# snipsco/sda

Measured on AMD Instinct MI355X. Metric: share-gen + clerk-sum elements/sec (mod q), higher is better.
Workload: dtype u64

## Files before the change

### sda_amd/csrc/clerk_sum.hpp

```cpp
#pragma once
#include <stddef.h>
#include <stdint.h>
#include <hip/hip_runtime.h>

#include "modarith.hpp"

namespace sda {

typedef long long ll2 __attribute__((ext_vector_type(2)));

template <bool VEC, int UNROLL>
__device__ __forceinline__ void combine_pair(uint64_t* __restrict__ acc_lo, int64_t* __restrict__ acc_hi,
                                             const int64_t* __restrict__ shares, size_t job_stride, size_t n_rows,
                                             size_t row_stride, size_t dimension, size_t rows_per_split, bool atomic,
                                             size_t pair, size_t by, size_t bz) {
    const size_t c0 = 2 * pair;
    if (c0 >= dimension) return;
    const bool two = c0 + 1 < dimension;
    const size_t job = by;
    const size_t r_begin = bz * rows_per_split;
    size_t r_end = r_begin + rows_per_split;
    if (r_end > n_rows) r_end = n_rows;
    const int64_t* base = shares + job * job_stride + c0;

    uint64_t lo0 = 0, lo1 = 0;
    int64_t hi0 = 0, hi1 = 0;
    size_t r = r_begin;
    if (VEC && two) {
        for (; r + UNROLL <= r_end; r += UNROLL) {
            ll2 v[UNROLL];
#pragma unroll
            for (int u = 0; u < UNROLL; ++u)
                v[u] = __builtin_nontemporal_load(reinterpret_cast<const ll2*>(base + (r + u) * row_stride));
#pragma unroll
            for (int u = 0; u < UNROLL; ++u) { acc_add(lo0, hi0, v[u].x); acc_add(lo1, hi1, v[u].y); }
        }
        for (; r < r_end; ++r) {
            ll2 v = __builtin_nontemporal_load(reinterpret_cast<const ll2*>(base + r * row_stride));
            acc_add(lo0, hi0, v.x); acc_add(lo1, hi1, v.y);
        }
    } else {
        for (; r < r_end; ++r) {
            acc_add(lo0, hi0, base[r * row_stride]);
            if (two) acc_add(lo1, hi1, base[r * row_stride + 1]);
        }
    }

    const size_t idx = job * dimension + c0;
    if (atomic) {
        acc_atomic_add(acc_lo + idx, acc_hi + idx, lo0, hi0);
        if (two) acc_atomic_add(acc_lo + idx + 1, acc_hi + idx + 1, lo1, hi1);
    } else {
        uint64_t l = acc_lo[idx]; int64_t h = acc_hi[idx];
        uint64_t nl = l + lo0; h += hi0 + (nl < l ? 1 : 0);
        acc_lo[idx] = nl; acc_hi[idx] = h;
        if (two) {
            l = acc_lo[idx + 1]; h = acc_hi[idx + 1];
            nl = l + lo1; h += hi1 + (nl < l ? 1 : 0);
            acc_lo[idx + 1] = nl; acc_hi[idx + 1] = h;
        }
    }
}

}
```

### sda_amd/csrc/modarith.hpp

```cpp
#pragma once
#include <stdint.h>

#if defined(__HIPCC__)
#include <hip/hip_runtime.h>
#define SDA_HD __host__ __device__ __forceinline__
#define SDA_D __device__ __forceinline__
#else
#define SDA_HD inline
#define SDA_D inline
#endif

namespace sda {

typedef unsigned __int128 u128;

struct U128 {
    uint64_t lo, hi;
};

SDA_HD U128 mul64x64(uint64_t a, uint64_t b) {
#if defined(__HIP_DEVICE_COMPILE__)
    U128 r;
    r.lo = a * b;
    r.hi = __umul64hi(a, b);
    return r;
#else
    u128 p = (u128)a * b;
    return U128{(uint64_t)p, (uint64_t)(p >> 64)};
#endif
}

SDA_HD uint64_t mulhi64(uint64_t a, uint64_t b) {
#if defined(__HIP_DEVICE_COMPILE__)
    return __umul64hi(a, b);
#else
    return (uint64_t)(((u128)a * b) >> 64);
#endif
}

SDA_HD void mac128(U128& acc, uint64_t a, uint64_t b) {
    U128 p = mul64x64(a, b);
    uint64_t lo = acc.lo + p.lo;
    acc.hi += p.hi + (lo < acc.lo ? 1u : 0u);
    acc.lo = lo;
}

struct MontCtx {
    uint64_t p;
    uint64_t pinv;
    uint64_t r2;
};

SDA_HD uint64_t mont_redc(U128 T, uint64_t p, uint64_t pinv) {
    uint64_t m = T.lo * pinv;
    uint64_t t = T.hi + mulhi64(m, p) + (T.lo != 0 ? 1u : 0u);
    return t >= p ? t - p : t;
}

SDA_HD void mont_acc_condsub(U128& acc, uint64_t p) {
    if (acc.hi >= p) acc.hi -= p;
}

SDA_HD uint64_t barrett_mod64(uint64_t v, uint64_t m, uint64_t mu) {
    uint64_t qhat = mulhi64(v, mu);
    uint64_t r = v - qhat * m;
    if (r >= m) r -= m;
    if (r >= m) r -= m;
    return r;
}

SDA_HD uint64_t canon_i64(int64_t x, uint64_t m, uint64_t mu) {
    if ((uint64_t)x < m) return (uint64_t)x;
    if (x >= 0) return barrett_mod64((uint64_t)x, m, mu);
    uint64_t mag = (uint64_t)0 - (uint64_t)x;
    uint64_t r = barrett_mod64(mag, m, mu);
    return r == 0 ? 0 : m - r;
}

SDA_HD uint64_t addmod(uint64_t a, uint64_t b, uint64_t m) {
    uint64_t s = a + b;
    return s >= m ? s - m : s;
}

SDA_HD uint64_t submod(uint64_t a, uint64_t b, uint64_t m) {
    return a >= b ? a - b : a + m - b;
}

SDA_HD uint64_t mod_i128(uint64_t lo, int64_t hi, uint64_t m, uint64_t mu) {
    bool neg = hi < 0;
    uint64_t mh = (uint64_t)hi, ml = lo;
    if (neg) {
        ml = ~ml + 1;
        mh = ~mh + (ml == 0 ? 1u : 0u);
    }
    uint64_t r = barrett_mod64(mh, m, mu);
    for (int i = 63; i >= 0; --i) {
        r = (r << 1) | ((ml >> i) & 1u);
        if (r >= m) r -= m;
    }
    return (neg && r != 0) ? m - r : r;
}

#if defined(__HIPCC__)
SDA_D void acc_add(uint64_t& lo, int64_t& hi, int64_t v) {
    const uint64_t nl = lo + (uint64_t)v;
    hi += (v >> 63) + (nl < lo ? 1 : 0);
    lo = nl;
}
SDA_D void acc_atomic_add(uint64_t* lo_p, int64_t* hi_p, uint64_t lo, int64_t hi) {
    if (lo != 0) {
        const unsigned long long old = atomicAdd(reinterpret_cast<unsigned long long*>(lo_p), (unsigned long long)lo);
        if (old + lo < old) hi += 1;
    }
    if (hi != 0) atomicAdd(reinterpret_cast<unsigned long long*>(hi_p), (unsigned long long)hi);
}
#endif

SDA_HD bool lemire_sample(uint64_t x, uint64_t m, uint64_t lemire_thr, uint64_t& out) {
    U128 pr = mul64x64(x, m);
    out = pr.hi;
    return pr.lo >= lemire_thr;
}

static constexpr uint64_t kDrbgPairedMax = 0x7F7F7Full;
SDA_HD bool drbg_paired(uint64_t m) { return m <= kDrbgPairedMax; }
SDA_HD bool lemire_pair(uint64_t x, uint32_t m, uint64_t thr2, uint32_t& ra, uint32_t& rb) {
    const uint64_t t0 = (uint64_t)(uint32_t)x * m;
    const uint64_t t1 = (uint64_t)(uint32_t)(x >> 32) * m + (t0 >> 32);
    ra = (uint32_t)(t1 >> 32);
    const uint64_t u0 = (uint64_t)(uint32_t)t0 * m;
    const uint64_t u1 = (uint64_t)(uint32_t)t1 * m + (u0 >> 32);
    rb = (uint32_t)(u1 >> 32);
    return ((u1 << 32) | (uint32_t)u0) >= thr2;
}

inline uint64_t h_mulmod(uint64_t a, uint64_t b, uint64_t m) { return (uint64_t)(((u128)a * b) % m); }

inline uint64_t h_powmod(uint64_t b, uint64_t e, uint64_t m) {
    uint64_t r = 1 % m;
    b %= m;
    while (e) {
        if (e & 1) r = h_mulmod(r, b, m);
        b = h_mulmod(b, b, m);
        e >>= 1;
    }
    return r;
}

inline bool h_invmod(uint64_t a, uint64_t m, uint64_t& out) {
    __int128 r0 = m, r1 = a % m, t0 = 0, t1 = 1;
    while (r1 != 0) {
        __int128 q = r0 / r1;
        __int128 r2 = r0 - q * r1; r0 = r1; r1 = r2;
        __int128 t2 = t0 - q * t1; t0 = t1; t1 = t2;
    }
    if (r0 != 1) return false;
    if (t0 < 0) t0 += m;
    out = (uint64_t)t0;
    return true;
}

inline uint64_t h_canon(int64_t x, uint64_t m) {
    __int128 r = (__int128)x % (__int128)m;
    if (r < 0) r += m;
    return (uint64_t)r;
}

inline uint64_t h_barrett_mu(uint64_t m) {
    return (uint64_t)((((u128)1) << 64) / m);
}

inline uint64_t h_lemire_thr(uint64_t m) {
    return (uint64_t)((((u128)1) << 64) % m);
}
inline uint64_t h_lemire_thr2(uint64_t m) {
    return drbg_paired(m) ? (uint64_t)((((u128)1) << 64) % ((u128)m * m)) : 0;
}

inline MontCtx h_mont_ctx(uint64_t p) {
    MontCtx c;
    c.p = p;
    uint64_t inv = p;
    for (int i = 0; i < 6; ++i) inv *= 2 - p * inv;
    c.pinv = (uint64_t)0 - inv;
    u128 r = (((u128)1) << 64) % p;
    c.r2 = (uint64_t)((r * r) % p);
    return c;
}

inline uint64_t h_to_mont(uint64_t x, uint64_t p) {
    return (uint64_t)((((u128)x) << 64) % p);
}

}
```

### sda_amd/csrc/ngemm_kernels.hip

```cpp
#include <hip/hip_runtime.h>
#include <stdint.h>

#include "capi_internal.hpp"
#include "chacha.hpp"
#include "clerk_sum.hpp"
#include "drbg_lane.hpp"
#include "kernels.hpp"
#include "launch_plan.hpp"
#include "modarith.hpp"

namespace sda {

typedef int ng_v4i __attribute__((ext_vector_type(4)));
typedef unsigned int ng_v4u __attribute__((ext_vector_type(4)));
typedef unsigned int ng_v2u __attribute__((ext_vector_type(2)));

static constexpr int kNgCompute = 8;
static constexpr int kNgWorkers = 64 * kNgCompute;
#ifndef NG_CLERK_WAVES
#define NG_CLERK_WAVES 3
#endif
static constexpr int kNgClerkWaves = NG_CLERK_WAVES;
static constexpr int kNgThreads = kNgWorkers + 64 + 64 * kNgClerkWaves;
typedef __attribute__((address_space(3))) uint8_t* ng_lptr;
// ... 125 lines not shown
        chacha_block_lane<20>(kk, (uint32_t)I, (uint32_t)(I >> 32), (uint32_t)stream, (uint32_t)(stream >> 32) & 0xFFFFFFu, o);
        const uint32_t i0 = 2u * j, i1 = i0 + 1u;
        const bool w0 = i0 >= d_lo, w1 = i1 < d_hi;
#pragma unroll
        for (int jj = 0; jj < 8; ++jj) {
            const int cc = jj >> 1, e = jj & 1;
            const uint64_t xw = ((uint64_t)o[8 * e + cc] << 32) | o[8 * e + 4 + cc];
            uint32_t ra, rb;
            if (!lemire_pair(xw, (uint32_t)m, thr2, ra, rb)) rej |= 1ull << (8u * round + (uint32_t)jj);
            if (w0) ng_put(B, WGB, 8u * nb + jj, k + i0 - t_lo, ng_digits(ra));
            if (w1) ng_put(B, WGB, 8u * nb + jj, k + i1 - t_lo, ng_digits(rb));
        }
    }
    if (__builtin_expect(rej != 0, 0)) ng_draw_fixup<WGB>(Bt, key, stream, b0, k, t, t_lo, d_lo, cd, m, thr2, rej);
}

template <int WGB>
__device__ __noinline__ void ng_direct_pass(const uint8_t* Bt, int64_t* op, size_t stride_clerk, uint64_t b0, uint64_t batches, uint32_t k,
                                            uint32_t t_lo, uint32_t d_lo, uint32_t d_hi) {
    const uint32_t lane = threadIdx.x & 63u, wave = threadIdx.x >> 6;
    const uint32_t o_lo = (k + d_lo - t_lo) & ~3u, o_hi = k + d_hi - t_lo;
    for (uint32_t bg = 0; bg < (uint32_t)(WGB / 64); ++bg) {
        const uint32_t bl = 64u * bg + lane;
        const uint64_t b = b0 + bl;
        const __attribute__((address_space(3))) uint8_t* q = (const __attribute__((address_space(3))) uint8_t*)Bt + bl * kNgRow;
        typedef const __attribute__((address_space(3))) uint32_t* lw;
        for (uint32_t o = o_lo + 4u * wave; o < o_hi; o += 4u * (uint32_t)kNgCompute) {
            const uint32_t w0 = *(lw)(q + o);
            const uint32_t w1 = *(lw)(q + WGB * kNgRow + o);
            const uint32_t w2 = *(lw)(q + 2 * WGB * kNgRow + o);
#pragma unroll
            for (int j = 0; j < 4; ++j) {
                const uint32_t v = (uint32_t)((int32_t)(int8_t)(w0 >> (8 * j)) + 256 * (int32_t)(int8_t)(w1 >> (8 * j)) +
                                              65536 * (int32_t)(int8_t)(w2 >> (8 * j)));
                const uint32_t term = t_lo + o + (uint32_t)j;
                if (b < batches && term >= k + d_lo && term < k + d_hi)
                    __builtin_nontemporal_store((long long)v, (__attribute__((address_space(1))) long long*)(op + (size_t)(term - k) * stride_clerk + b));
            }
        }
    }
}

template <int KS, int NT, int STEP>
__device__ __forceinline__ void ng_stage(ng_v4i (&bfrag)[NT][KS > 1 ? NgBSource<KS>::in_regs : 1][3], uint8_t* Bt, uint8_t* Side, const GenLayout& L, const ModParams& mod, const DrbgKey& key,
                                         const NGemmPlan& P, const int64_t* sp, const int64_t* rp, int64_t* op, uint64_t stream, uint64_t b0,
                                         uint64_t batches
#ifdef NG_TIMING
                                         , uint64_t (&ng_tm)[4]
#endif
                                         ) {
    constexpr int WB = 16 * NT, WGB = kNgCompute * WB;
    const uint32_t lane = threadIdx.x & 63u, wave = threadIdx.x >> 6, col = lane & 15u, g = lane >> 4;
    const uint32_t k = P.k, t = P.t, kt = k + t, t_lo = 64u * STEP;
    const bool worker = wave < (uint32_t)kNgCompute;
    const bool loads = t_lo < k || rp != nullptr || t_lo + 64u > kt;
    const bool draws_here = !rp && t_lo + 64u > k && t_lo < kt;
    const uint32_t d_lo = t_lo > k ? t_lo - k : 0u, d_hi = draws_here ? (t_lo + 64u < kt ? t_lo + 64u : kt) - k : d_lo;
#ifdef NG_TIMING
    const uint64_t tq0 = __builtin_readcyclecounter();
#endif
    if (worker) {
        if (loads) ng_load_pass<WGB>(Bt, sp, rp, L.len, batches, b0, k, t, t_lo, mod.m, mod.mu);
#ifdef NG_TIMING
        ng_tm[0] += __builtin_readcyclecounter() - tq0;
#endif
        if (draws_here) ng_draw_pass<WGB>(Bt, key, stream, b0, k, t, t_lo, d_lo, d_hi - d_lo, mod.m, mod.lemire_thr2);
    }
#ifdef NG_TIMING
    const uint64_t tq1 = __builtin_readcyclecounter();
#endif
    __syncthreads();
#ifdef NG_TIMING
    const uint64_t tq2 = __builtin_readcyclecounter();
    ng_tm[1] += tq1 - tq0; ng_tm[2] += tq2 - tq1;
#endif
    if (worker) {
        if (draws_here && L.direct_rows) ng_direct_pass<WGB>(Bt, op, L.out_stride_clerk, b0, batches, k, t_lo, d_lo, d_hi);
#ifdef NG_TIMING
        ng_tm[3] += __builtin_readcyclecounter() - tq2;
#endif
        if constexpr (STEP < NgBSource<KS>::in_regs || (NgBSource<KS>::stash && STEP == KS - 2)) {
#pragma unroll
            for (int nt = 0; nt < NT; ++nt)
#pragma unroll
                for (int lb = 0; lb < 3; ++lb) {
                    const ng_v4i f = *reinterpret_cast<const ng_v4i*>(Bt + ((size_t)lb * WGB + wave * WB + NT * col + nt) * kNgRow + 16 * g);
                    if constexpr (STEP < NgBSource<KS>::in_regs) bfrag[nt][STEP][lb] = f;
                    else *reinterpret_cast<ng_v4i*>(Side + ((size_t)(wave * NT + nt) * 3 + lb) * 1024 + lane * 16) = f;
                }
        }
    }
    __syncthreads();
#ifdef NG_TIMING
    if constexpr (STEP + 1 < KS) ng_stage<KS, NT, STEP + 1>(bfrag, Bt, Side, L, mod, key, P, sp, rp, op, stream, b0, batches, ng_tm);
#else
    if constexpr (STEP + 1 < KS) ng_stage<KS, NT, STEP + 1>(bfrag, Bt, Side, L, mod, key, P, sp, rp, op, stream, b0, batches);
#endif
}

struct NgFuse {
    uint64_t* acc_lo; int64_t* acc_hi; const int64_t* prev;
    size_t job_stride, n_rows, row_stride, dimension, rows_per_split;
    uint32_t col_blocks, jobs, splits, pad;
    uint64_t n_gen, n_comb, n_comb_wg, period;
    uint64_t n_early;
    uint32_t items_per_wg;
    uint32_t pad2;
    uint64_t cw_items, cw_per_slot;
    uint64_t* cw_progress;
    uint32_t cw_col_blocks, cw_pad;
};
static constexpr int kNgClerkUnroll = 8;
static constexpr int kNgClerkUnrollShort = 20;

template <int KS> struct NgRing { static constexpr int depth = KS == 8 ? 2 : 4; };

__device__ __forceinline__ void ng_store_guard(ng_v4u v) { asm volatile("s_nop 1" ::"v"(v)); }
__device__ __forceinline__ void ng_store_guard(ng_v2u v) { asm volatile("s_nop 1" ::"v"(v)); }

struct NgClerkCursor {
    uint64_t it, end;
    uint64_t job; uint32_t bx;
    uint32_t r;
};
static constexpr int kNgClerkRows = 10;

struct NgClerkSet {
    ll2 v[kNgClerkRows];
    ll2 al, ah;
};

__device__ __forceinline__ void ng_clerk_advance(NgClerkCursor& c, uint32_t n_rows, uint32_t col_blocks) {
    c.r += kNgClerkRows;
    if (c.r >= n_rows) {
        c.r = 0; ++c.it;
        if (++c.bx == col_blocks) { c.bx = 0; ++c.job; }
    }
}
__device__ __forceinline__ void ng_clerk_load(ll2& dst, const void* p) {
    asm volatile("global_load_dwordx4 %0, %1, off nt ; NGCL" : "=v"(dst) : "v"(p) : "memory");
}
__device__ __forceinline__ void ng_clerk_load_plain(ll2& dst, const void* p) {
    asm volatile("global_load_dwordx4 %0, %1, off ; NGCL" : "=v"(dst) : "v"(p) : "memory");
}
template <int YOUNGER>
__device__ __forceinline__ void ng_clerk_wait(NgClerkSet& S) {
    static_assert(kNgClerkRows == 10, "the operand list below names ten rows");
    asm volatile("s_waitcnt vmcnt(%12) ; NGCW %0 %1 %2 %3 %4 %5 %6 %7 %8 %9 %10 %11"
                 : "+v"(S.v[0]), "+v"(S.v[1]), "+v"(S.v[2]), "+v"(S.v[3]), "+v"(S.v[4]), "+v"(S.v[5]), "+v"(S.v[6]), "+v"(S.v[7]),
                   "+v"(S.v[8]), "+v"(S.v[9]), "+v"(S.al), "+v"(S.ah)
                 : "n"(YOUNGER)
                 : "memory");
}

__device__ __forceinline__ void ng_clerk_wave(const NgFuse& F, uint64_t slot, uint32_t lane, uint32_t n_barriers, uint32_t extra) {
    if (F.cw_items == 0) {
        for (uint32_t b = 0; b < n_barriers; ++b) __builtin_amdgcn_s_barrier();
        return;
    }
    const uint32_t n_rows = (uint32_t)F.n_rows, col_blocks = F.cw_col_blocks;
    NgClerkCursor is, cs;
    is.it = slot * F.cw_per_slot < F.cw_items ? slot * F.cw_per_slot : F.cw_items;
    is.end = is.it + F.cw_per_slot < F.cw_items ? is.it + F.cw_per_slot : F.cw_items;
    is.job = is.it / col_blocks; is.bx = (uint32_t)(is.it - is.job * col_blocks); is.r = 0;
    cs = is;
    uint64_t lo0 = 0, lo1 = 0, bl0 = 0, bl1 = 0;
    int64_t hi0 = 0, hi1 = 0, bh0 = 0, bh1 = 0;
    NgClerkSet A, B;
    bool validA = false, validB = false;
    auto issue = [&](NgClerkSet& S, bool& valid) {
        valid = is.it < is.end;
        size_t c0 = 2 * ((size_t)is.bx * 64 + lane);
        if (c0 + 1 >= F.dimension) c0 = 0;
        const uint64_t job = valid ? is.job : 0;
        const uint32_t r0 = valid ? is.r : 0;
        const int64_t* base = F.prev + job * F.job_stride + c0;
        if (valid && r0 == 0) {
            const size_t idx = job * F.dimension + c0;
            ng_clerk_load_plain(S.al, F.acc_lo + idx);
            ng_clerk_load_plain(S.ah, F.acc_hi + idx);
        }
#pragma unroll
        for (int u = 0; u < kNgClerkRows; ++u) {
            const uint32_t rr = r0 + u < n_rows ? r0 + u : n_rows - 1;
            ng_clerk_load(S.v[u], base + (size_t)rr * F.row_stride);
        }
        if (valid) ng_clerk_advance(is, n_rows, col_blocks);
    };
    auto flush = [&]() {
        const size_t c0 = 2 * ((size_t)cs.bx * 64 + lane);
        if (c0 + 1 >= F.dimension) return;
        const size_t idx = cs.job * F.dimension + c0;
        const uint64_t n0 = bl0 + lo0, n1 = bl1 + lo1;
        ll2 l, h;
        l.x = (long long)n0; l.y = (long long)n1;
        h.x = bh0 + hi0 + (n0 < bl0 ? 1 : 0); h.y = bh1 + hi1 + (n1 < bl1 ? 1 : 0);
        *reinterpret_cast<ll2*>(F.acc_lo + idx) = l;
        *reinterpret_cast<ll2*>(F.acc_hi + idx) = h;
    };
    auto consume = [&](NgClerkSet& S, bool& valid) {
        if (!valid) return;
        valid = false;
        if (cs.r == 0) {
            bl0 = (uint64_t)S.al.x; bl1 = (uint64_t)S.al.y; bh0 = S.ah.x; bh1 = S.ah.y;
            lo0 = lo1 = 0; hi0 = hi1 = 0;
        }
#pragma unroll
        for (int u = 0; u < kNgClerkRows; ++u)
            if (cs.r + u < n_rows) { acc_add(lo0, hi0, S.v[u].x); acc_add(lo1, hi1, S.v[u].y); }
        if (cs.r + kNgClerkRows >= n_rows) flush();
        ng_clerk_advance(cs, n_rows, col_blocks);
    };
#pragma unroll
    for (int u = 0; u < kNgClerkRows; ++u) { A.v[u] = ll2{0, 0}; B.v[u] = ll2{0, 0}; }
    A.al = A.ah = B.al = B.ah = ll2{0, 0};
    uint32_t b = 0;
    for (; b + 1 < n_barriers; b += 2) {
        const uint32_t e = b < 32u ? (extra >> b) & 3u : 0u;
        if (e >= 1u) {
            ng_clerk_wait<kNgClerkRows>(A);
            consume(A, validA); issue(A, validA);
            ng_clerk_wait<kNgClerkRows>(B);
            consume(B, validB); issue(B, validB);
        }
        if (e >= 2u) {
            ng_clerk_wait<kNgClerkRows>(A);
            consume(A, validA); issue(A, validA);
            ng_clerk_wait<kNgClerkRows>(B);
            consume(B, validB); issue(B, validB);
        }
        ng_clerk_wait<kNgClerkRows>(A);
        consume(A, validA); issue(A, validA);
        __builtin_amdgcn_s_barrier();
        ng_clerk_wait<kNgClerkRows>(B);
        consume(B, validB); issue(B, validB);
        __builtin_amdgcn_s_barrier();
    }
    if (b < n_barriers) {
        ng_clerk_wait<kNgClerkRows>(A);
        consume(A, validA); issue(A, validA);
        __builtin_amdgcn_s_barrier();
        ng_clerk_wait<0>(B); consume(B, validB);
        ng_clerk_wait<0>(A); consume(A, validA);
    } else {
        ng_clerk_wait<0>(A); consume(A, validA);
        ng_clerk_wait<0>(B); consume(B, validB);
    }
    if (cs.it < cs.end && cs.r != 0) flush();
    if (F.cw_progress && lane == 0) { F.cw_progress[2 * slot] = cs.it; F.cw_progress[2 * slot + 1] = cs.r; }
}

static constexpr int kNgClerkRest = 16;
__global__ __launch_bounds__(64) void ngemm_clerk_rest_kernel(NgFuse F, uint64_t slots) {
    const uint32_t lane = threadIdx.x, n_rows = (uint32_t)F.n_rows;
    for (uint64_t slot = blockIdx.x; slot < slots; slot += gridDim.x) {
        uint64_t it = F.cw_progress[2 * slot];
        uint32_t r0 = (uint32_t)F.cw_progress[2 * slot + 1];
        const uint64_t first = slot * F.cw_per_slot < F.cw_items ? slot * F.cw_per_slot : F.cw_items;
        const uint64_t end = first + F.cw_per_slot < F.cw_items ? first + F.cw_per_slot : F.cw_items;
        for (; it < end; ++it, r0 = 0) {
            const uint64_t job = it / F.cw_col_blocks, bx = it - job * F.cw_col_blocks;
            const size_t c0 = 2 * ((size_t)bx * 64 + lane);
            if (c0 >= F.dimension) continue;
            const bool two = c0 + 1 < F.dimension;
            const int64_t* base = F.prev + job * F.job_stride + c0;
            const size_t idx = job * F.dimension + c0;
            const uint64_t l0 = F.acc_lo[idx], l1 = two ? F.acc_lo[idx + 1] : 0;
            const int64_t h0 = F.acc_hi[idx], h1 = two ? F.acc_hi[idx + 1] : 0;
            uint64_t lo0 = 0, lo1 = 0;
            int64_t hi0 = 0, hi1 = 0;
            for (uint32_t r = r0; r < n_rows; r += kNgClerkRest) {
                ll2 v[kNgClerkRest];
#pragma unroll
                for (int u = 0; u < kNgClerkRest; ++u) {
                    const uint32_t rr = r + u < n_rows ? r + u : n_rows - 1;
                    v[u] = __builtin_nontemporal_load(reinterpret_cast<const ll2*>(base + (size_t)rr * F.row_stride));
                }
#pragma unroll
                for (int u = 0; u < kNgClerkRest; ++u)
                    if (r + u < n_rows) { acc_add(lo0, hi0, v[u].x); if (two) acc_add(lo1, hi1, v[u].y); }
            }
            uint64_t nl = l0 + lo0;
            F.acc_lo[idx] = nl; F.acc_hi[idx] = h0 + hi0 + (nl < l0 ? 1 : 0);
            if (two) { nl = l1 + lo1; F.acc_lo[idx + 1] = nl; F.acc_hi[idx + 1] = h1 + hi1 + (nl < l1 ? 1 : 0); }
        }
    }
}

template <int N> __device__ __forceinline__ void ng_wait_vm() { asm volatile("s_waitcnt vmcnt(%0)" ::"n"(N) : "memory"); }

template <int KS>
__device__ __noinline__ void ng_loader_rows(const uint8_t* A, uint8_t* Abuf, uint32_t tiles, uint32_t lane) {
    constexpr int PIECES = KS * 3, ATILE = PIECES * 1024, DEPTH = NgRing<KS>::depth;
    auto issue_tile = [&](uint32_t tile, uint32_t slot) {
        const uint8_t* src = A + (size_t)tile * ATILE + lane * 16;
        uint8_t* dst = Abuf + slot * ATILE;
#pragma unroll
        for (int q = 0; q < PIECES; ++q)
            __builtin_amdgcn_global_load_lds((const __attribute__((address_space(1))) void*)(src + q * 1024),
                                             (__attribute__((address_space(3))) void*)(dst + q * 1024), 16, 0, 0);
    };
    uint32_t slot = DEPTH - 1;
    for (uint32_t rt = 0; rt < tiles; ++rt) {
        const uint32_t nxt = rt + DEPTH - 1;
        if (nxt < tiles) {
            issue_tile(nxt, slot);
            ng_wait_vm<PIECES * (DEPTH - 2) < 63 ? PIECES * (DEPTH - 2) : 0>();
        } else {
            ng_wait_vm<0>();
        }
        slot = slot + 1 == (uint32_t)DEPTH ? 0u : slot + 1;
        __builtin_amdgcn_s_barrier();
    }
}

template <int KS, int NT>
__global__ __launch_bounds__(kNgThreads) __attribute__((amdgpu_waves_per_eu(3, 3))) void packed_gen_ngemm_kernel(GenLayout L, ModParams mod, DrbgKey key, NGemmPlan P,
                                                                        uint64_t chunks, uint64_t batches, NgFuse F) {
    constexpr int WB = 16 * NT, WGB = kNgCompute * WB;
    constexpr int PIECES = KS * 3, ATILE = PIECES * 1024;
    constexpr int DEPTH = NgRing<KS>::depth;
    extern __shared__ __align__(16) uint8_t ng_lds[];
    uint8_t* Abuf = ng_lds;
    uint8_t* Bt = ng_lds + DEPTH * ATILE;
    uint8_t* Side = Bt + 3 * WGB * kNgRow;
    const uint32_t tid = threadIdx.x, lane = tid & 63u, wave = tid >> 6, col = lane & 15u, g = lane >> 4;
    uint64_t item = blockIdx.x;
    auto role_at = [&](uint64_t pos, uint64_t& idx) -> int {
        if (!F.n_comb_wg) { idx = pos; return pos < (uint64_t)gridDim.x ? 0 : 2; }
        const uint64_t mixed = F.n_gen + F.n_early;
        if (pos >= mixed) { idx = F.n_early + (pos - mixed); return idx < F.n_comb_wg ? 1 : 2; }
        const uint64_t q = pos / F.period, rem = pos - q * F.period;
        if (rem == 0 && q < F.n_early) { idx = q; return 1; }
        const uint64_t before = q + (rem ? 1 : 0);
        idx = pos - (before < F.n_early ? before : F.n_early);
        return idx < F.n_gen ? 0 : 2;
    };
    {
        uint64_t idx;
        const int role = role_at(item, idx);
        if (role == 2) return;
        if (role == 1) {
            if (tid < 512u) {
                const uint64_t first = idx * F.items_per_wg + (tid >> 8);
                for (uint32_t j = 0; j < F.items_per_wg; j += 2) {
                    const uint64_t it = first + j;
                    if (it >= F.n_comb) break;
                    const uint64_t bx = it % F.col_blocks, rest = it / F.col_blocks;
                    if (F.rows_per_split % kNgClerkUnrollShort == 0 && F.rows_per_split <= 4 * kNgClerkUnrollShort)
                        combine_pair<true, kNgClerkUnrollShort>(F.acc_lo, F.acc_hi, F.prev, F.job_stride, F.n_rows, F.row_stride, F.dimension,
                                                                F.rows_per_split, F.splits > 1, bx * 256u + (tid & 255u), rest % F.jobs, rest / F.jobs);
                    else
                        combine_pair<true, kNgClerkUnroll>(F.acc_lo, F.acc_hi, F.prev, F.job_stride, F.n_rows, F.row_stride, F.dimension,
                                                           F.rows_per_split, F.splits > 1, bx * 256u + (tid & 255u), rest % F.jobs, rest / F.jobs);
                }
            }
            return;
        }
        item = idx;
    }
    if (wave > (uint32_t)kNgCompute) {
        const uint32_t cw = __builtin_amdgcn_readfirstlane(wave) - (uint32_t)kNgCompute - 1u;
        uint32_t extra = 0;
        if (!L.rand) {
#pragma unroll
            for (int st = 0; st < KS; ++st) {
                const uint32_t lo = 64u * st > P.k ? 64u * st : P.k, hi = 64u * st + 64u < P.k + P.t ? 64u * st + 64u : P.k + P.t;
                const uint32_t draws = hi > lo ? hi - lo : 0u;
                extra |= (draws >= 48u ? 2u : draws >= 24u ? 1u : 0u) << (2 * st);
            }
        }
        ng_clerk_wave(F, item * (uint64_t)kNgClerkWaves + cw, lane, 2u * (uint32_t)KS + P.row_tiles, extra);
        return;
    }
    const uint64_t p = item / chunks, chunk = item - p * chunks;
    const uint64_t b0 = chunk * WGB;
    const int64_t* sp = L.secrets + p * L.secrets_stride;
    const int64_t* rp = L.rand ? L.rand + p * L.rand_stride : nullptr;
    const uint64_t stream = L.first_participant + p;
    const uint32_t tiles = P.row_tiles;
    const bool loader = wave == (uint32_t)kNgCompute;
    auto issue_tile = [&](uint32_t tile, uint32_t slot) {
        const uint8_t* src = P.A + (size_t)tile * ATILE + lane * 16;
        uint8_t* dst = Abuf + slot * ATILE;
#pragma unroll
        for (int q = 0; q < PIECES; ++q)
            __builtin_amdgcn_global_load_lds((const __attribute__((address_space(1))) void*)(src + q * 1024),
                                             (__attribute__((address_space(3))) void*)(dst + q * 1024), 16, 0, 0);
    };
    if (loader) {
        for (uint32_t tile = 0; tile < (uint32_t)(DEPTH - 1) && tile < tiles; ++tile) issue_tile(tile, tile);
        ng_wait_vm<0>();
    }

#if defined(NG_TIMING) || defined(NG_PHASES)
    const uint64_t ng_t0 = __builtin_readcyclecounter();
    const uint64_t ng_w0 = wall_clock64();
#endif
    ng_v4i bfrag[NT][KS > 1 ? NgBSource<KS>::in_regs : 1][3];
    int64_t* op = L.out + p * L.out_stride_participant;
#ifdef NG_TIMING
    uint64_t ng_tm[4] = {0, 0, 0, 0};
    ng_stage<KS, NT, 0>(bfrag, Bt, Side, L, mod, key, P, sp, rp, op, stream, b0, batches, ng_tm);
    const uint64_t ng_t1 = __builtin_readcyclecounter();
#else
    ng_stage<KS, NT, 0>(bfrag, Bt, Side, L, mod, key, P, sp, rp, op, stream, b0, batches);
#endif
#ifdef NG_PHASES
    const uint64_t ng_t1 = __builtin_readcyclecounter();
#endif

    if (loader) {
        ng_loader_rows<KS>(P.A, Abuf, tiles, lane);
        return;
    }
    const uint32_t bl = wave * WB + (uint32_t)NT * col;
    const uint64_t obase_v = reinterpret_cast<uint64_t>(op + b0 + (size_t)(rp ? 0u : L.direct_rows) * L.out_stride_clerk);
    const uint32_t obase_hi = (uint32_t)__builtin_amdgcn_readfirstlane((uint32_t)(obase_v >> 32));
    const uint32_t obase_lo = (uint32_t)__builtin_amdgcn_readfirstlane((uint32_t)obase_v);
    const char* obase = reinterpret_cast<const char*>(((uint64_t)obase_hi << 32) | (uint64_t)obase_lo);
    const size_t row_bytes = L.out_stride_clerk * sizeof(int64_t);
    const uint32_t loff = bl * 8u + 4u * g * (uint32_t)row_bytes;
    const bool late = wave >= (uint32_t)(kNgCompute / 2);
    constexpr int KREG = NgBSource<KS>::in_regs, NLDS = KS - KREG;
    auto step_at = [](int pos) constexpr {
        if (NLDS == 2) return pos == 0 ? 0 : pos == 1 ? KS - 2 : pos == 2 ? 1 : pos == 3 ? KS - 1 : pos - 2;
        return pos;
    };
    ng_v4i acc[NT][5];
    auto products = [&](uint32_t slot_) {
        constexpr int GROUPS = KS * 3;
        const uint8_t* Acur = Abuf + slot_ * ATILE + (size_t)lane * 16;
        uint32_t bt_off = (wave * WB + NT * col) * kNgRow + 16u * g;
        uint32_t st_off = wave * NT * 3u * 1024u + lane * 16u;
        asm volatile("" : "+v"(bt_off), "+v"(st_off));
        ng_v4i bl[NT][3];
        auto fetch_b = [&](int ks) {
// ... 40 lines not shown
        S = ng_mad(c2, acc[nt][2][i], S);
        S = ng_mad(c3, top, S);
        return ng_redc(S, P.np);
    };
    auto finish_whole = [&](uint32_t rt) {
        char* tbase = const_cast<char*>(obase) + (size_t)rt * 16u * row_bytes;
        const __amdgpu_buffer_rsrc_t rs = __builtin_amdgcn_make_buffer_rsrc(tbase, 0, 0xFFFFFFFFu, 0x00020000);
        if constexpr (NT == 1) {
#pragma unroll
            for (int i = 0; i < 4; ++i) {
                const ng_v2u v = {reduce1(0, i), 0u};
                __builtin_amdgcn_raw_buffer_store_b64(v, rs, loff, (uint32_t)i * (uint32_t)row_bytes, 2);
                ng_store_guard(v);
            }
        } else {
#pragma unroll
            for (int nt = 0; nt < NT; nt += 2) {
                uint32_t even[4];
#pragma unroll
                for (int i = 0; i < 4; ++i) even[i] = reduce1(nt, i);
#pragma unroll
                for (int i = 0; i < 4; ++i) {
                    const ng_v4u v = {even[i], 0u, reduce1(nt + 1, i), 0u};
                    const __amdgpu_buffer_rsrc_t rsi = __builtin_amdgcn_make_buffer_rsrc(tbase + (size_t)i * row_bytes, 0, 0xFFFFFFFFu, 0x00020000);
                    __builtin_amdgcn_raw_buffer_store_b128(v, rsi, loff + 8 * nt, 0, 2);
                    ng_store_guard(v);
                }
            }
        }
    };
    const uint32_t lim = b0 + bl >= batches ? 0u : (batches - b0 - bl > (uint64_t)NT ? (uint32_t)NT : (uint32_t)(batches - b0 - bl));
    auto finish_masked = [&](uint32_t rt) {
        const __amdgpu_buffer_rsrc_t rs = __builtin_amdgcn_make_buffer_rsrc(const_cast<char*>(obase) + (size_t)rt * 16u * row_bytes, 0, 0xFFFFFFFFu, 0x00020000);
        const uint32_t row0 = 16u * rt + 4u * g;
#pragma unroll
        for (int nt = 0; nt < NT; ++nt)
#pragma unroll
            for (int i = 0; i < 4; ++i) {
                const ng_v2u v = {reduce1(nt, i), 0u};
                if ((uint32_t)nt < lim && row0 + (uint32_t)i < P.n) {
                    __builtin_amdgcn_raw_buffer_store_b64(v, rs, loff + 8 * nt, (uint32_t)i * (uint32_t)row_bytes, 2);
                    ng_store_guard(v);
                }
            }
    };
    auto finish_far = [&](uint32_t rt) {
        uint32_t gg = g, bb = bl;
        asm volatile("" : "+v"(gg), "+v"(bb));
        const uint32_t row0 = 16u * rt + 4u * gg;
#pragma unroll
        for (int nt = 0; nt < NT; ++nt)
#pragma unroll
            for (int i = 0; i < 4; ++i) {
                const uint32_t v = reduce1(nt, i);
                if ((uint32_t)nt < lim && row0 + (uint32_t)i < P.n)
                    __builtin_nontemporal_store((long long)v, reinterpret_cast<long long*>(const_cast<char*>(obase) + (size_t)(row0 + (uint32_t)i) * row_bytes) + bb + nt);
            }
    };
    const uint32_t whole_tiles = whole ? (P.n / 16u < tiles ? P.n / 16u : tiles) : 0u;
    auto finish = [&](uint32_t rt) {
        c0 = ng_pin_vgpr(P.c[0]); c1 = ng_pin_vgpr(P.c[1]); c2 = ng_pin_vgpr(P.c[2]); c3 = ng_pin_vgpr(P.c[3]);
        if (rt < whole_tiles) finish_whole(rt); else if (near) finish_masked(rt); else finish_far(rt);
        __builtin_amdgcn_sched_barrier(0);
    };
    uint32_t slot = 0;
    for (uint32_t rt = 0; rt < tiles; ++rt) {
        if (late && rt) finish(rt - 1);
        products(slot);
        slot = slot + 1 == (uint32_t)DEPTH ? 0u : slot + 1;
        if (!late) finish(rt);
        __syncthreads();
    }
    if (late && tiles) finish(tiles - 1);
#ifdef NG_PHASES
    if (tid == 0) {
        int64_t* o = L.out + p * L.out_stride_participant + b0;
        o[0] = (int64_t)(ng_t1 - ng_t0);
        o[1] = (int64_t)(__builtin_readcyclecounter() - ng_t1);
        o[6] = (int64_t)ng_w0; o[7] = (int64_t)wall_clock64();
    }
#endif
#ifdef NG_TIMING
    if (tid == 0) {
        int64_t* o = L.out + p * L.out_stride_participant + b0;
        o[0] = (int64_t)(ng_t1 - ng_t0);
        o[1] = (int64_t)(__builtin_readcyclecounter() - ng_t1);
        o[2] = (int64_t)ng_tm[0]; o[3] = (int64_t)ng_tm[1]; o[4] = (int64_t)ng_tm[2]; o[5] = (int64_t)ng_tm[3];
        o[6] = (int64_t)ng_w0; o[7] = (int64_t)wall_clock64();
    }
    if (lane == 0) {
        int64_t* o = L.out + p * L.out_stride_participant + b0 + 8 + 4 * wave;
        o[0] = (int64_t)ng_tm[0]; o[1] = (int64_t)ng_tm[1]; o[2] = (int64_t)ng_tm[2]; o[3] = (int64_t)ng_tm[3];
    }
#endif
}

static constexpr uint64_t kNgPrimeMax = 0x7F7F7Full;
static_assert(kNgPrimeMax == kDrbgPairedMax, "the limb GEMM draws with the paired rule for every prime it accepts");
bool packed_ngemm_path_available(uint32_t k, uint32_t t, uint64_t p) {
    return k >= 1 && k + t >= 1 && k + t <= 512 && p <= kNgPrimeMax && drbg_paired(p);
}
uint32_t packed_ngemm_steps(uint32_t k, uint32_t t) {
    const uint32_t need = (k + t + 63) / 64;
    return need <= 1 ? 1u : need <= 2 ? 2u : need <= 4 ? 4u : 8u;
}

size_t ngemm_tile_bytes(uint32_t ks) { return (size_t)ks * 3 * 1024; }

static uint32_t ng_cu_count() {
    int dev = 0, n = 0;
    if (hipGetDevice(&dev) != hipSuccess || hipDeviceGetAttribute(&n, hipDeviceAttributeMultiprocessorCount, dev) != hipSuccess) {
        (void)hipGetLastError();
        return 0;
    }
    return n > 0 ? (uint32_t)n : 0u;
}

template <int KS, int NT>
static hipError_t ngemm_launch(const GenLayout& L, const ModParams& mod, const DrbgKey& key, const NGemmPlan& P, hipStream_t s) {
    constexpr int WGB = 16 * kNgCompute * NT;
    const uint64_t batches = (L.len + P.k - 1) / P.k;
    const uint64_t chunks = (batches + WGB - 1) / WGB;
    if (chunks * L.participants == 0) return hipSuccess;
    const size_t lds = ngemm_lds_bytes<KS, NT>();
    auto kern = packed_gen_ngemm_kernel<KS, NT>;
    if (lds > 64 * 1024)
        if (hipError_t e = hipFuncSetAttribute(reinterpret_cast<const void*>(kern), hipFuncAttributeMaxDynamicSharedMemorySize, (int)lds)) return e;
    return for_participant_slices(L, chunks, kMaxBlocksI31, [&](const GenLayout& S, uint64_t blocks) {
        note_kernel("packed_gen_ngemm_kernel<%d, %d>", KS, NT);
        kern<<<dim3((unsigned)blocks), dim3(kNgThreads), lds, s>>>(S, mod, key, P, chunks, batches, NgFuse{});
        return hipGetLastError();
    });
}

hipError_t launch_packed_generate_ngemm(const GenLayout& L, const ModParams& mod, const DrbgKey& key, const NGemmPlan& P, hipStream_t s) {
    switch (P.ks) {
        case 1: return ngemm_launch<1, 4>(L, mod, key, P, s);
        case 2: return ngemm_launch<2, 2>(L, mod, key, P, s);
        case 4: return ngemm_launch<4, 2>(L, mod, key, P, s);
        case 8: return ngemm_launch<8, 1>(L, mod, key, P, s);
        default: return hipErrorInvalidValue;
    }
}

template <int KS, int NT>
static hipError_t ngemm_launch_fused(const GenLayout& L, const ModParams& mod, const DrbgKey& key, const NGemmPlan& P, NgFuse F,
                                     size_t prev_rows, hipStream_t s, bool* fused, uint64_t* d_progress, size_t progress_slots) {
    constexpr int WGB = 16 * kNgCompute * NT;
    const uint64_t batches = (L.len + P.k - 1) / P.k;
    const uint64_t chunks = (batches + WGB - 1) / WGB;
    F.n_gen = chunks * L.participants;
    const bool have_comb = F.prev && prev_rows > 0 && F.jobs > 0 && F.dimension > 0;
    const uint64_t slots = F.n_gen * (uint64_t)kNgClerkWaves;
    if (d_progress && have_comb && F.n_gen > 0 && F.n_gen <= 0x7FFFFFFFull && slots <= progress_slots && prev_rows < (1ull << 31) &&
        F.dimension % 2 == 0) {
        const uint64_t col_blocks = (((F.dimension + 1) / 2) + 63) / 64;
        if (col_blocks <= 0xFFFFFFFFull) {
            F.cw_col_blocks = (uint32_t)col_blocks;
            F.cw_items = col_blocks * F.jobs;
            F.cw_per_slot = (F.cw_items + slots - 1) / slots;
            F.cw_progress = d_progress;
            F.n_comb = 0; F.n_comb_wg = 0; F.n_early = 0; F.period = 1; F.items_per_wg = 0;
            const size_t lds = ngemm_lds_bytes<KS, NT>();
            auto kern = packed_gen_ngemm_kernel<KS, NT>;
            if (lds > 64 * 1024)
                if (hipError_t e = hipFuncSetAttribute(reinterpret_cast<const void*>(kern), hipFuncAttributeMaxDynamicSharedMemorySize, (int)lds)) return e;
            *fused = true;
            note_kernel("packed_gen_ngemm_kernel<%d, %d>", KS, NT);
            kern<<<dim3((unsigned)F.n_gen), dim3(kNgThreads), lds, s>>>(L, mod, key, P, chunks ? chunks : 1, batches, F);
            if (hipError_t e = hipGetLastError()) return e;
            const uint64_t cap = 256ull * 32ull;
            ngemm_clerk_rest_kernel<<<dim3((unsigned)(slots < cap ? slots : cap)), dim3(64), 0, s>>>(F, slots);
            return hipGetLastError();
        }
    }
    F.col_blocks = (uint32_t)((((F.dimension + 1) / 2) + 255) / 256);
    uint64_t splits = have_comb ? (prev_rows + 511) / 512 : 1;
    if (splits > 64) splits = 64;
    F.rows_per_split = have_comb ? (prev_rows + splits - 1) / splits : 1;
    splits = have_comb ? (prev_rows + F.rows_per_split - 1) / F.rows_per_split : 1;
    F.splits = (uint32_t)splits;
    F.n_comb = have_comb ? (uint64_t)F.col_blocks * F.jobs * splits : 0;
    uint64_t per_wg = 2;
    const uint64_t most = F.n_gen == 0 ? (~0ull >> 2) : (F.n_gen / 2 ? F.n_gen / 2 : 1);
    if ((F.n_comb + 1) / 2 > most) per_wg = 2 * ((F.n_comb + 2 * most - 1) / (2 * most));
    if (per_wg > 0xFFFFFFFEull) return hipSuccess;
    F.items_per_wg = (uint32_t)per_wg;
    F.n_comb_wg = (F.n_comb + per_wg - 1) / per_wg;
    const uint32_t cus = ng_cu_count() ? ng_cu_count() : 256u;
    const uint64_t late = F.n_gen < 16ull * cus ? F.n_comb_wg / 3 : 0;
    F.n_early = F.n_comb_wg - late;
    F.period = F.n_early ? F.n_gen / F.n_early + 1 : 1;
    if (F.n_early && (F.period & 1) == 0) F.period = F.period > 2 ? F.period - 1 : 3;
    uint64_t grid = F.n_gen + F.n_comb_wg;
    if (F.n_early && (F.n_early - 1) * F.period + 1 > F.n_gen + F.n_early) return hipSuccess;
    if (grid == 0) { *fused = true; return hipSuccess; }
    if (grid > 0x7FFFFFFFull) return hipSuccess;
    if (F.n_comb_wg == 0) { *fused = true; return ngemm_launch<KS, NT>(L, mod, key, P, s); }
    const size_t lds = ngemm_lds_bytes<KS, NT>();
    auto kern = packed_gen_ngemm_kernel<KS, NT>;
    if (lds > 64 * 1024)
        if (hipError_t e = hipFuncSetAttribute(reinterpret_cast<const void*>(kern), hipFuncAttributeMaxDynamicSharedMemorySize, (int)lds)) return e;
    *fused = true;
    note_kernel("packed_gen_ngemm_kernel<%d, %d>", KS, NT);
    kern<<<dim3((unsigned)grid), dim3(kNgThreads), lds, s>>>(L, mod, key, P, chunks ? chunks : 1, batches, F);
    return hipGetLastError();
}

uint64_t ngemm_clerk_slots(const GenLayout& L, const NGemmPlan& P) {
    const int nt = P.ks == 1 ? 4 : P.ks == 8 ? 1 : 2;
    const uint64_t wgb = 16ull * kNgCompute * nt, batches = (L.len + P.k - 1) / P.k;
    return (batches + wgb - 1) / wgb * L.participants * (uint64_t)kNgClerkWaves;
}

hipError_t launch_fused_packed_ngemm(const GenLayout& L, const ModParams& mod, const DrbgKey& key, const NGemmPlan& P,
                                     const ClerkSumTarget& C, hipStream_t s, bool* fused, uint64_t* d_progress, size_t progress_slots) {
    *fused = false;
    if (L.rand) return hipSuccess;
    if (L.participants == 0 || L.len == 0) return hipSuccess;
    const bool have_comb = C.prev && C.prev_rows > 0 && C.jobs > 0 && C.dimension > 0;
    if (have_comb && !(aligned16(C.prev) && (L.out_stride_clerk % 2 == 0) && (L.out_stride_participant % 2 == 0)))
        return hipSuccess;
    NgFuse F{};
    F.acc_lo = C.acc_lo; F.acc_hi = C.acc_hi; F.prev = C.prev;
    F.job_stride = L.out_stride_clerk; F.row_stride = L.out_stride_participant;
    F.n_rows = C.prev_rows; F.dimension = C.dimension; F.jobs = (uint32_t)C.jobs;
    switch (P.ks) {
        case 1: return ngemm_launch_fused<1, 4>(L, mod, key, P, F, C.prev_rows, s, fused, d_progress, progress_slots);
        case 2: return ngemm_launch_fused<2, 2>(L, mod, key, P, F, C.prev_rows, s, fused, d_progress, progress_slots);
        case 4: return ngemm_launch_fused<4, 2>(L, mod, key, P, F, C.prev_rows, s, fused, d_progress, progress_slots);
        case 8: return ngemm_launch_fused<8, 1>(L, mod, key, P, F, C.prev_rows, s, fused, d_progress, progress_slots);
        default: return hipErrorInvalidValue;
    }
}

}
```

Before: 117.3 billion.

## Accumulate clerk sums as split 32-bit halves with mad_u64 instructions

Replaces the per-element 128-bit carry-tracking add with two 64-bit accumulators of the 32-bit low and high halves, each updated by a single v_mad_u64_u32 or v_mad_i64_i32. The halves are folded into the 128-bit result only once per chunk of at most 2^31 rows, so no carry compare is needed per element. Row-bound predicates become a scalar multiplier instead of branches. The clerk wave loop also settles outstanding loads explicitly at the end. This trims VALU work in the share-summing loops, at the cost of inline asm and row-count limits tied to overflow safety.

Result: no change. 116.9 billion (-0.4%).

```diff
diff --git a/sda_amd/csrc/clerk_sum.hpp b/sda_amd/csrc/clerk_sum.hpp
--- a/sda_amd/csrc/clerk_sum.hpp
+++ b/sda_amd/csrc/clerk_sum.hpp
@@ -23,43 +23,51 @@
     if (r_end > n_rows) r_end = n_rows;
     const int64_t* base = shares + job * job_stride + c0;
 
-    uint64_t lo0 = 0, lo1 = 0;
-    int64_t hi0 = 0, hi1 = 0;
-    size_t r = r_begin;
-    if (VEC && two) {
-        for (; r + UNROLL <= r_end; r += UNROLL) {
-            ll2 v[UNROLL];
+    const size_t idx = job * dimension + c0;
+    size_t r_next = r_begin;
+    do {
+        size_t r = r_next;
+        const size_t r_stop = r + kHalvesMaxRows < r_end ? r + kHalvesMaxRows : r_end;
+        r_next = r_stop;
+        HalfSums s0, s1;
+        if (VEC && two) {
+            for (; r + UNROLL <= r_stop; r += UNROLL) {
+                ll2 v[UNROLL];
 #pragma unroll
-            for (int u = 0; u < UNROLL; ++u)
-                v[u] = __builtin_nontemporal_load(reinterpret_cast<const ll2*>(base + (r + u) * row_stride));
+                for (int u = 0; u < UNROLL; ++u)
+                    v[u] = __builtin_nontemporal_load(reinterpret_cast<const ll2*>(base + (r + u) * row_stride));
 #pragma unroll
-            for (int u = 0; u < UNROLL; ++u) { acc_add(lo0, hi0, v[u].x); acc_add(lo1, hi1, v[u].y); }
+                for (int u = 0; u < UNROLL; ++u) { s0.add(v[u].x); s1.add(v[u].y); }
+            }
+            for (; r < r_stop; ++r) {
+                ll2 v = __builtin_nontemporal_load(reinterpret_cast<const ll2*>(base + r * row_stride));
+                s0.add(v.x); s1.add(v.y);
+            }
+        } else {
+            for (; r < r_stop; ++r) {
+                s0.add(base[r * row_stride]);
+                if (two) s1.add(base[r * row_stride + 1]);
+            }
         }
-        for (; r < r_end; ++r) {
-            ll2 v = __builtin_nontemporal_load(reinterpret_cast<const ll2*>(base + r * row_stride));
-            acc_add(lo0, hi0, v.x); acc_add(lo1, hi1, v.y);
+        uint64_t lo0 = 0, lo1 = 0;
+        int64_t hi0 = 0, hi1 = 0;
+        s0.fold_into(lo0, hi0);
+        s1.fold_into(lo1, hi1);
+
+        if (atomic) {
+            acc_atomic_add(acc_lo + idx, acc_hi + idx, lo0, hi0);
+            if (two) acc_atomic_add(acc_lo + idx + 1, acc_hi + idx + 1, lo1, hi1);
+        } else {
+            uint64_t l = acc_lo[idx]; int64_t h = acc_hi[idx];
+            uint64_t nl = l + lo0; h += hi0 + (nl < l ? 1 : 0);
+            acc_lo[idx] = nl; acc_hi[idx] = h;
+            if (two) {
+                l = acc_lo[idx + 1]; h = acc_hi[idx + 1];
+                nl = l + lo1; h += hi1 + (nl < l ? 1 : 0);
+                acc_lo[idx + 1] = nl; acc_hi[idx + 1] = h;
+            }
         }
-    } else {
-        for (; r < r_end; ++r) {
-            acc_add(lo0, hi0, base[r * row_stride]);
-            if (two) acc_add(lo1, hi1, base[r * row_stride + 1]);
-        }
-    }
-
-    const size_t idx = job * dimension + c0;
-    if (atomic) {
-        acc_atomic_add(acc_lo + idx, acc_hi + idx, lo0, hi0);
-        if (two) acc_atomic_add(acc_lo + idx + 1, acc_hi + idx + 1, lo1, hi1);
-    } else {
-        uint64_t l = acc_lo[idx]; int64_t h = acc_hi[idx];
-        uint64_t nl = l + lo0; h += hi0 + (nl < l ? 1 : 0);
-        acc_lo[idx] = nl; acc_hi[idx] = h;
-        if (two) {
-            l = acc_lo[idx + 1]; h = acc_hi[idx + 1];
-            nl = l + lo1; h += hi1 + (nl < l ? 1 : 0);
-            acc_lo[idx + 1] = nl; acc_hi[idx + 1] = h;
-        }
-    }
+    } while (r_next < r_end);
 }
 
 }
diff --git a/sda_amd/csrc/modarith.hpp b/sda_amd/csrc/modarith.hpp
--- a/sda_amd/csrc/modarith.hpp
+++ b/sda_amd/csrc/modarith.hpp
@@ -101,7 +101,37 @@
     return (neg && r != 0) ? m - r : r;
 }
 
+static constexpr uint64_t kHalvesMaxRows = 1ull << 31;
+SDA_HD void halves_fold(uint64_t& lo, int64_t& hi, uint64_t L, int64_t H) {
+    const uint64_t v = L + ((uint64_t)H << 32);
+    const uint64_t nl = lo + v;
+    hi += (H >> 32) + (v < L ? 1 : 0) + (nl < lo ? 1 : 0);
+    lo = nl;
+}
+
 #if defined(__HIPCC__)
+struct HalfSums {
+    uint64_t L = 0;
+    int64_t H = 0;
+    SDA_D void add(int64_t v) {
+        asm("v_mad_u64_u32 %0, vcc, 1, %1, %0" : "+v"(L) : "v"((uint32_t)v) : "vcc");
+        asm("v_mad_i64_i32 %0, vcc, 1, %1, %0" : "+v"(H) : "v"((int32_t)(v >> 32)) : "vcc");
+    }
+    SDA_D void add_if(int64_t v, uint32_t m) {
+        asm("v_mad_u64_u32 %0, vcc, %1, %2, %0" : "+v"(L) : "s"(m), "v"((uint32_t)v) : "vcc");
+        asm("v_mad_i64_i32 %0, vcc, %1, %2, %0" : "+v"(H) : "s"(m), "v"((int32_t)(v >> 32)) : "vcc");
+    }
+    SDA_D void fold_into(uint64_t& lo, int64_t& hi) {
+        halves_fold(lo, hi, L, H);
+        L = 0; H = 0;
+    }
+};
+SDA_D uint32_t uniform_lt(uint32_t a, uint32_t b) {
+    uint32_t m;
+    asm("s_cmp_lt_u32 %1, %2\n\ts_cselect_b32 %0, 1, 0" : "=s"(m) : "s"(a), "s"(b) : "scc");
+    return m;
+}
+
 SDA_D void acc_add(uint64_t& lo, int64_t& hi, int64_t v) {
     const uint64_t nl = lo + (uint64_t)v;
     hi += (v >> 63) + (nl < lo ? 1 : 0);
diff --git a/sda_amd/csrc/ngemm_kernels.hip b/sda_amd/csrc/ngemm_kernels.hip
--- a/sda_amd/csrc/ngemm_kernels.hip
+++ b/sda_amd/csrc/ngemm_kernels.hip
@@ -301,6 +301,14 @@
                  : "n"(YOUNGER)
                  : "memory");
 }
+__device__ __forceinline__ void ng_clerk_settle(NgClerkSet& S) {
+    static_assert(kNgClerkRows == 10, "the operand list below names ten rows");
+    asm volatile("s_waitcnt vmcnt(0)"
+                 : "+v"(S.v[0]), "+v"(S.v[1]), "+v"(S.v[2]), "+v"(S.v[3]), "+v"(S.v[4]), "+v"(S.v[5]), "+v"(S.v[6]), "+v"(S.v[7]),
+                   "+v"(S.v[8]), "+v"(S.v[9]), "+v"(S.al), "+v"(S.ah)
+                 :
+                 : "memory");
+}
 
 __device__ __forceinline__ void ng_clerk_wave(const NgFuse& F, uint64_t slot, uint32_t lane, uint32_t n_barriers, uint32_t extra) {
     if (F.cw_items == 0) {
@@ -313,8 +321,9 @@
     is.end = is.it + F.cw_per_slot < F.cw_items ? is.it + F.cw_per_slot : F.cw_items;
     is.job = is.it / col_blocks; is.bx = (uint32_t)(is.it - is.job * col_blocks); is.r = 0;
     cs = is;
-    uint64_t lo0 = 0, lo1 = 0, bl0 = 0, bl1 = 0;
-    int64_t hi0 = 0, hi1 = 0, bh0 = 0, bh1 = 0;
+    HalfSums s0, s1;
+    uint64_t bl0 = 0, bl1 = 0;
+    int64_t bh0 = 0, bh1 = 0;
     NgClerkSet A, B;
     bool validA = false, validB = false;
     auto issue = [&](NgClerkSet& S, bool& valid) {
@@ -337,13 +346,13 @@
         if (valid) ng_clerk_advance(is, n_rows, col_blocks);
     };
     auto flush = [&]() {
+        s0.fold_into(bl0, bh0); s1.fold_into(bl1, bh1);
         const size_t c0 = 2 * ((size_t)cs.bx * 64 + lane);
         if (c0 + 1 >= F.dimension) return;
         const size_t idx = cs.job * F.dimension + c0;
-        const uint64_t n0 = bl0 + lo0, n1 = bl1 + lo1;
         ll2 l, h;
-        l.x = (long long)n0; l.y = (long long)n1;
-        h.x = bh0 + hi0 + (n0 < bl0 ? 1 : 0); h.y = bh1 + hi1 + (n1 < bl1 ? 1 : 0);
+        l.x = (long long)bl0; l.y = (long long)bl1;
+        h.x = bh0; h.y = bh1;
         *reinterpret_cast<ll2*>(F.acc_lo + idx) = l;
         *reinterpret_cast<ll2*>(F.acc_hi + idx) = h;
     };
@@ -352,11 +361,13 @@
         valid = false;
         if (cs.r == 0) {
             bl0 = (uint64_t)S.al.x; bl1 = (uint64_t)S.al.y; bh0 = S.ah.x; bh1 = S.ah.y;
-            lo0 = lo1 = 0; hi0 = hi1 = 0;
-        }
-#pragma unroll
-        for (int u = 0; u < kNgClerkRows; ++u)
-            if (cs.r + u < n_rows) { acc_add(lo0, hi0, S.v[u].x); acc_add(lo1, hi1, S.v[u].y); }
+            s0 = HalfSums(); s1 = HalfSums();
+        }
+#pragma unroll
+        for (int u = 0; u < kNgClerkRows; ++u) {
+            const uint32_t m = uniform_lt(cs.r + u, n_rows);
+            s0.add_if(S.v[u].x, m); s1.add_if(S.v[u].y, m);
+        }
         if (cs.r + kNgClerkRows >= n_rows) flush();
         ng_clerk_advance(cs, n_rows, col_blocks);
     };
@@ -364,7 +375,7 @@
     for (int u = 0; u < kNgClerkRows; ++u) { A.v[u] = ll2{0, 0}; B.v[u] = ll2{0, 0}; }
     A.al = A.ah = B.al = B.ah = ll2{0, 0};
     uint32_t b = 0;
-    for (; b + 1 < n_barriers; b += 2) {
+    if (n_barriers >= 2) for (;; b += 2) {
         const uint32_t e = b < 32u ? (extra >> b) & 3u : 0u;
         if (e >= 1u) {
             ng_clerk_wait<kNgClerkRows>(A);
@@ -384,6 +395,11 @@
         ng_clerk_wait<kNgClerkRows>(B);
         consume(B, validB); issue(B, validB);
         __builtin_amdgcn_s_barrier();
+        if (b + 3 >= n_barriers) {
+            ng_clerk_settle(A); ng_clerk_settle(B);
+            b += 2;
+            break;
+        }
     }
     if (b < n_barriers) {
         ng_clerk_wait<kNgClerkRows>(A);
@@ -414,10 +430,9 @@
             const bool two = c0 + 1 < F.dimension;
             const int64_t* base = F.prev + job * F.job_stride + c0;
             const size_t idx = job * F.dimension + c0;
-            const uint64_t l0 = F.acc_lo[idx], l1 = two ? F.acc_lo[idx + 1] : 0;
-            const int64_t h0 = F.acc_hi[idx], h1 = two ? F.acc_hi[idx + 1] : 0;
-            uint64_t lo0 = 0, lo1 = 0;
-            int64_t hi0 = 0, hi1 = 0;
+            uint64_t l0 = F.acc_lo[idx], l1 = two ? F.acc_lo[idx + 1] : 0;
+            int64_t h0 = F.acc_hi[idx], h1 = two ? F.acc_hi[idx + 1] : 0;
+            HalfSums s0, s1;
             for (uint32_t r = r0; r < n_rows; r += kNgClerkRest) {
                 ll2 v[kNgClerkRest];
 #pragma unroll
@@ -426,12 +441,14 @@
                     v[u] = __builtin_nontemporal_load(reinterpret_cast<const ll2*>(base + (size_t)rr * F.row_stride));
                 }
 #pragma unroll
-                for (int u = 0; u < kNgClerkRest; ++u)
-                    if (r + u < n_rows) { acc_add(lo0, hi0, v[u].x); if (two) acc_add(lo1, hi1, v[u].y); }
+                for (int u = 0; u < kNgClerkRest; ++u) {
+                    const uint32_t m = uniform_lt(r + u, n_rows);
+                    s0.add_if(v[u].x, m); s1.add_if(v[u].y, m);
+                }
             }
-            uint64_t nl = l0 + lo0;
-            F.acc_lo[idx] = nl; F.acc_hi[idx] = h0 + hi0 + (nl < l0 ? 1 : 0);
-            if (two) { nl = l1 + lo1; F.acc_lo[idx + 1] = nl; F.acc_hi[idx + 1] = h1 + hi1 + (nl < l1 ? 1 : 0); }
+            s0.fold_into(l0, h0); s1.fold_into(l1, h1);
+            F.acc_lo[idx] = l0; F.acc_hi[idx] = h0;
+            if (two) { F.acc_lo[idx + 1] = l1; F.acc_hi[idx + 1] = h1; }
         }
     }
 }
@@ -778,7 +795,8 @@
     F.n_gen = chunks * L.participants;
     const bool have_comb = F.prev && prev_rows > 0 && F.jobs > 0 && F.dimension > 0;
     const uint64_t slots = F.n_gen * (uint64_t)kNgClerkWaves;
-    if (d_progress && have_comb && F.n_gen > 0 && F.n_gen <= 0x7FFFFFFFull && slots <= progress_slots && prev_rows < (1ull << 31) &&
+    static_assert(kHalvesMaxRows <= 1ull << 31, "the kernels also hold a row index in 32 bits and add to it");
+    if (d_progress && have_comb && F.n_gen > 0 && F.n_gen <= 0x7FFFFFFFull && slots <= progress_slots && prev_rows < kHalvesMaxRows &&
         F.dimension % 2 == 0) {
         const uint64_t col_blocks = (((F.dimension + 1) / 2) + 63) / 64;
         if (col_blocks <= 0xFFFFFFFFull) {
```
